# nucypher/TFHE.jl

Measured on AMD Instinct MI355X. Metric: bootstrapped gates/sec (whole node), N=1024, higher is better.
Workload: dtype int32 torus / f64 transform; 1 GPU; batch of 4096 independent gate_nand() bootstraps per GPU, tfhe_parameters_80 (n=500, N=1024, k=1, l=2, Bg=2^10, ks t=8, base 2^2); inputs=resident in HBM, launch=one process

## Files before the change

### tfhe.jl_amd/csrc/engine_dispatch.hip

```cpp
#define TFHE_EMIT_KEYSWITCH_KERNELS
#include "engine.hpp"
#include "br_launch.hpp"

#include <map>
#include <mutex>
#include <functional>

int32_t ensure_dyn_lds(tfhe_ctx *c, const void *fn, size_t bytes, const char *what)
{
    static std::mutex mu;
    static std::map<std::pair<int, const void *>, size_t> have;
    std::lock_guard<std::mutex> lk(mu);
    size_t &cur = have[std::make_pair(c->device, fn)];
    if (cur >= bytes) return TFHE_OK;
    const hipError_t e = hipFuncSetAttribute(fn, hipFuncAttributeMaxDynamicSharedMemorySize, (int)bytes);
    if (e != hipSuccess) return c->set_err(TFHE_ERR_DEVICE, "hipFuncSetAttribute(%s, %zu bytes of LDS) failed: %s", what, bytes, hipGetErrorString(e));
    cur = bytes;
    return TFHE_OK;
}

int32_t prepare_diag(tfhe_ctx *c, size_t R, hipStream_t s, DiagArgs &d)
{
    d.margin_bits = nullptr; d.clk = nullptr; d.phase = nullptr;
    c->diag_rows = 0;
    if (!c->measure_margin) return TFHE_OK;
    HIP_TRY(c, c->diag.reserve(R * 24 + 64 * 8));
    HIP_TRY(c, hipMemsetAsync(c->diag.p, 0, R * 24 + 64 * 8, s));
    d.margin_bits = (unsigned long long *)c->diag.p;
    d.clk = d.margin_bits + R;
    d.phase = d.clk + 2 * R;
    c->diag_rows = R;
    return TFHE_OK;
}

void name_kernel(tfhe_ctx *c, const char *fmt, ...)
{
    char buf[128];
    va_list ap;
    va_start(ap, fmt);
    vsnprintf(buf, sizeof buf, fmt, ap);
    va_end(ap);
    c->last_kernel = buf;
}

static int br_inst_l(const tfhe_ctx *c)
{
    return (c->P.bs_l == 2 || c->P.bs_l == 3) && !c->br_rt_l ? c->P.bs_l : 0;
}

static void name_br(tfhe_ctx *c, const char *family, int L, const char *rest = "")
{
    if (L) name_kernel(c, "blind_rotate_kernel_%s<%d%s>", family, L, rest);
    else name_kernel(c, "blind_rotate_kernel_%s<0%s>(l=%d)", family, rest, c->P.bs_l);
}

static int32_t launch_blind_rotate_part(tfhe_ctx *c, size_t first, size_t R, int32_t mu, hipStream_t s, const DiagArgs &diag, int k2_kind = -1 ,
                                        const TvPtrs *tv_all = nullptr)
{
    TvPtrs tv{nullptr, nullptr};
    if (tv_all) tv = TvPtrs{tv_all->tv, tv_all->index + first, tv_all->bodies ? tv_all->bodies + first * (size_t)tv_all->n_out : nullptr, tv_all->n_out};
    BrArgs a;
    a.diag = diag;
    if (diag.margin_bits) { a.diag.margin_bits += first; a.diag.clk += 2 * first; }
    const bool dg = c->measure_margin;
    a.bara = (const int32_t *)c->bara.p + first * (size_t)(c->P.n + 1);
    a.bk = c->d_bk;
    a.ext = (int32_t *)c->ext.p + first * ((size_t)c->P.k * c->P.N + 1);
    a.T = c->T;
    a.tan2 = reinterpret_cast<const double *>(c->d_tables + kTan2TableOffset);
    a.g = c->g;
    a.n = c->P.n;
    a.mu = mu;
    a.prio_steps = (int32_t)((int64_t)c->P.n * c->br_prio_pct / 100);
    a.R = (int32_t)R;
    const int L = c->P.bs_l;
    a.l = L;
    if (c->anyn()) {
        const int K1 = c->P.k + 1, N = c->P.N, M = N / 2;
        anyn::Args g;
        g.diag = a.diag; g.bara = a.bara; g.bk = a.bk; g.ext = a.ext; g.g = c->g; g.n = a.n; g.mu = mu; g.K1 = K1; g.L = L; g.R = (int32_t)R;
        g.log2N = ilog2i(N); g.parties = 1;
        g.wtab = c->d_anyn_tab; g.twist = c->d_anyn_tab + M;
        HIP_TRY(c, c->mk_acc.reserve((first + R) * (size_t)K1 * N * sizeof(int32_t)));
        g.acc = (int32_t *)c->mk_acc.p + first * (size_t)K1 * N;
        const bool fits = anyn::lds_bytes(N, K1) <= 160 * 1024;
        const bool spec_lds = c->anyn_spec < 0 ? fits : (c->anyn_spec == 0 && fits);
        g.spec_g = nullptr;
        if (!spec_lds) {
            HIP_TRY(c, c->spec.reserve((first + R) * (size_t)K1 * (M > 0 ? M : 1) * sizeof(cplx)));
            g.spec_g = (cplx *)c->spec.p + first * (size_t)K1 * (M > 0 ? M : 1);
        }
        const BrLaunch geo{0, 1, dg, dim3((unsigned)R), dim3((unsigned)anyn::threads_for(N)), anyn::lds_bytes(N, spec_lds ? K1 : 0)};
        const int32_t rc = tv_all ? br_launch_anyn(c, with_tv(g, tv), geo, s) : br_launch_anyn(c, g, geo, s);
        if (rc) return rc;
        name_kernel(c, spec_lds ? "blind_rotate_kernel_anyn(N=%d,k=%d,l=%d)" : "blind_rotate_kernel_anyn(N=%d,k=%d,l=%d,spec=global)", N, c->P.k, L);
        return TFHE_OK;
    }
    if (c->n512()) {
        N512Args b;
        b.diag = a.diag; b.bara = a.bara; b.bk = a.bk; b.ext = a.ext; b.g = c->g; b.n = a.n; b.mu = mu; b.R = (int32_t)R; b.l = L;
        b.prio_steps = a.prio_steps;
        b.tw1 = c->d_tables + kN512TableOffset; b.tw2q = c->d_tables + kH2TableOffset + 512; b.tw3q = b.tw2q + 64;
        if (c->n512_w2 == 1 || (c->n512_w2 < 0 && R <= 6 * (size_t)c->cu_count)) {
            const BrLaunch geo{br_inst_l(c), 1, dg, dim3((unsigned)R), dim3(128), kN512W2LdsBytes};
            const int32_t rc = tv_all ? br_launch_n512w2(c, with_tv(b, tv), geo, s) : br_launch_n512w2(c, b, geo, s);
            if (rc) return rc;
            name_br(c, "n512w2", geo.L);
            return TFHE_OK;
        }
        const bool group = !dg && (c->n512_rw == 4 || (c->n512_rw == 0 && R >= 8 * (size_t)c->cu_count));
        const int rw = group ? 4 : 1;
        const BrLaunch geo{br_inst_l(c), rw, dg, dim3((unsigned)((R + rw - 1) / rw)), dim3(64 * rw), (size_t)rw * kN512LdsBytes};
        const int32_t rc = tv_all ? br_launch_n512(c, with_tv(b, tv), geo, s) : br_launch_n512(c, b, geo, s);
        if (rc) return rc;
        name_br(c, "n512", geo.L, group ? ",rw4" : "");
        return TFHE_OK;
    }
    const bool tuned = c->P.N == kN2 ? (c->P.k == 1 && L == 3) : c->P.k == 1 ? true : (c->P.k == 2 && (L == 2 || L == 3));
    if (!tuned || c->br_general) {
        const int K1 = c->P.k + 1, H = c->P.N / kN;
        const size_t img = (size_t)kMir + c->P.N;
        BrGenArgs g;
        g.diag = a.diag; g.bara = a.bara; g.bk = a.bk; g.ext = a.ext; g.g = c->g; g.n = a.n; g.mu = mu; g.K1 = K1; g.L = L; g.R = (int32_t)R;
        HIP_TRY(c, c->mk_acc.reserve((first + R) * K1 * img * sizeof(int32_t)));
        g.acc = (int32_t *)c->mk_acc.p + first * K1 * img;
        g.tw1f = c->P.N == kN2 ? (const cplx *)(c->d_tables + kTableElems) : c->T.tw1f;
        g.tw2 = c->T.tw2;
        const BrLaunch geo{0, 1, dg, dim3((unsigned)R), dim3(64), (kXchElems + 64 + (size_t)K1 * H * kM) * sizeof(cplx)};
        const bool n2048 = c->P.N == kN2;
        const int32_t rc = tv_all ? br_launch_general(c, with_tv(g, tv), n2048, geo, s) : br_launch_general(c, g, n2048, geo, s);
        if (rc) return rc;
        name_kernel(c, "blind_rotate_kernel_general(N=%d,k=%d,l=%d)", c->P.N, c->P.k, L);
        return TFHE_OK;
    }
    if (c->P.N == kN2) {
        Br2048Args b;
        b.diag = a.diag; b.bara = a.bara; b.bk = a.bk; b.ext = a.ext; b.tw1f2 = c->d_tables + kTableElems; b.tw2 = c->T.tw2; b.g = c->g; b.n = a.n; b.mu = mu; b.prio_steps = a.prio_steps;
        b.R = (int32_t)R;
        const int rw = dg ? 1 : c->n2048_rw ? c->n2048_rw : (R <= (size_t)c->cu_count ? 1 : 2);
        const size_t ldsb = (size_t)rw * (2 * kImg2 * 4 + 2 * kXchElems * sizeof(cplx)) + 64 * sizeof(cplx) + 64;
        const BrLaunch geo{L, rw, dg, dim3((unsigned)((R + rw - 1) / rw)), dim3(128 * rw), ldsb};
        const int32_t rc = tv_all ? br_launch_n2048x(c, with_tv(b, tv), geo, s) : br_launch_n2048x(c, b, geo, s);
        if (rc) return rc;
        name_br(c, "n2048x", L, rw == 2 ? ",rw2" : ",rw1");
        return TFHE_OK;
    }
    if (c->P.k == 2) {
        const size_t cus = (size_t)c->cu_count;
        const bool w3 = k2_kind >= 0 ? k2_kind == 1 : (c->k2_w3 == 1 || (c->k2_w3 < 0 && R <= 2 * cus));
        if (w3) {
            const BrLaunch geo{L, 1, dg, dim3((unsigned)R), dim3(192), kK2W3LdsBytes};
            const int32_t rc = tv_all ? br_launch_k2w3(c, with_tv(a, tv), geo, s) : br_launch_k2w3(c, a, geo, s);
            if (rc) return rc;
            name_br(c, "k2w3", L);
            return TFHE_OK;
        }
        const bool grouped = !dg && (c->k2_rw == 7 || c->k2_rw == 0);
        size_t blocks = R;
        if (grouped) {
            const size_t rounds = (R + 7 * cus - 1) / (7 * cus);
            blocks = std::min(R, rounds * cus);
            a.grp_q = (int32_t)(R / blocks);
            a.grp_big = (int32_t)(R % blocks);
        }
        const int rw = grouped ? 7 : 1;
        const BrLaunch geo{L, rw, dg, dim3((unsigned)blocks), dim3(64 * rw), (size_t)rw * kK2LdsBytes};
        const int32_t rc = tv_all ? br_launch_k2(c, with_tv(a, tv), geo, s) : br_launch_k2(c, a, geo, s);
        if (rc) return rc;
        name_br(c, "k2", L, grouped ? ",rw7" : "");
        return TFHE_OK;
    }
    const int64_t tiny = c->br_tiny == -2 ? (int64_t)c->cu_count : c->br_tiny;
    if (tiny >= 0 && (int64_t)R <= tiny && (L == 2 || L == 3) && !c->br_rt_l) {
        H2Tables ht;
        ht.tw1h = c->d_tables + kH2TableOffset; ht.tw2q = ht.tw1h + 512; ht.tw3q = ht.tw2q + 64;
        const size_t ldsh = 2 * kImg * 4 + (size_t)4 * L * (kH2Buf + 256) * sizeof(cplx) + 2 * 2 * kN * 4;
        const BrLaunch geo{L, 1, dg, dim3((unsigned)R), dim3(256 * L), ldsh};
        const int32_t rc = tv_all ? br_launch_h2(c, with_tv(a, tv), ht, geo, s) : br_launch_h2(c, a, ht, geo, s);
        if (rc) return rc;
        name_br(c, "h2", L);
        return TFHE_OK;
    }
    if (c->br_small >= 0 && (int64_t)R <= c->br_small) {
        const size_t cus2 = 2 * (size_t)c->cu_count;
        const bool pairs = !dg && (c->w2_rw == 2 || (c->w2_rw == 0 && ((R > cus2 / 2 && R <= cus2) || R > 2 * cus2 - cus2 / 8)));
        const int rw = pairs ? 2 : 1;
        const BrLaunch geo{br_inst_l(c), rw, dg, dim3((unsigned)((R + rw - 1) / rw)), dim3(128 * rw), (size_t)rw * kW2LdsBytes};
        const int32_t rc = tv_all ? br_launch_w2(c, with_tv(a, tv), geo, s) : br_launch_w2(c, a, geo, s);
        if (rc) return rc;
        name_br(c, "w2", geo.L, pairs ? ",rw2" : "");
        return TFHE_OK;
    }
    const bool group = c->v3_rw == 4 || (c->v3_rw == 0 && R >= 6 * (size_t)c->cu_count);
    const int rw = group ? 4 : 1;
    const BrLaunch geo{br_inst_l(c), rw, dg, dim3((unsigned)((R + rw - 1) / rw)), dim3(64 * rw), (size_t)rw * kV3LdsBytes};
    const int32_t rc = tv_all ? br_launch_v3(c, with_tv(a, tv), geo, s) : br_launch_v3(c, a, geo, s);
    if (rc) return rc;
    name_br(c, "v3", geo.L, group ? ",8,tw2reg,rw4" : ",8,tw2reg");
    return TFHE_OK;
}

static const double kK2RoundCost[8] = {0.0, 6.8, 6.85, 7.2, 7.3, 9.45, 9.55, 10.3};
static const double kK2W3RoundCost[3] = {0.0, 3.1, 4.3};
struct K2Seg { size_t count; int kind; };
static std::vector<K2Seg> k2_partition(size_t R, size_t cus, bool allow_w3)
{
    const size_t q = (R + cus - 1) / cus;
    if (q <= 2 && allow_w3) return {{R, 1}};
    if (q <= 7 && !allow_w3) return {{R, 0}};
    std::vector<double> best(q + 1, 1e300);
    std::vector<int> take(q + 1, 0);
    best[0] = 0.0;
    for (size_t i = 1; i <= q; i++)
        for (int n = 1; n <= 7 && (size_t)n <= i; n++)
            if (best[i - n] + kK2RoundCost[n] < best[i]) { best[i] = best[i - n] + kK2RoundCost[n]; take[i] = n; }
    int tail = 0;
    double total = best[q];
    for (int t = 1; allow_w3 && t <= 2 && (size_t)t <= q; t++)
        if (best[q - t] + kK2W3RoundCost[t] < total) { total = best[q - t] + kK2W3RoundCost[t]; tail = t; }
    std::vector<int> rounds;
    for (size_t i = q - (size_t)tail; i > 0; i -= (size_t)take[i]) rounds.push_back(take[i]);
    std::sort(rounds.begin(), rounds.end(), std::greater<int>());
    std::vector<K2Seg> seg;
    size_t done = 0;
    for (size_t i = 0; i < rounds.size() && done < R;) {
        size_t j = i;
        while (j < rounds.size() && rounds[j] == rounds[i]) j++;
        const size_t want = (size_t)rounds[i] * (j - i) * cus;
        if ((j == rounds.size() && !tail) || done + want >= R) { seg.push_back({R - done, 0}); done = R; break; }
        seg.push_back({want, 0});
        done += want;
        i = j;
    }
    if (done < R) seg.push_back({R - done, 1});
    return seg;
}

int32_t launch_blind_rotate(tfhe_ctx *c, size_t R, int32_t mu, hipStream_t s, const TvPtrs *tv)
{
    if (tv && c->measure_margin) return c->set_err(TFHE_ERR_STATE, "bootstrap_tv: no DIAG instantiation of the TV kernels (measure_margin is on)");
    DiagArgs diag;
    int32_t rc = prepare_diag(c, R, s, diag);
    if (rc) return rc;
    alloc_checkpoint();
    std::vector<K2Seg> seg;
    const bool tuned_l = c->P.bs_l == 2 || c->P.bs_l == 3;
    if (c->anyn()) {
    } else if (c->br_split && !c->br_general && !c->measure_margin && c->P.N == kN && c->P.k == 2 && tuned_l && (c->k2_rw == 0 || c->k2_rw == 7) && c->k2_w3 != 1) {
        seg = k2_partition(R, (size_t)c->cu_count, c->k2_w3 < 0);
    } else if (c->br_split && !c->br_general && c->P.N == kN && c->P.k == 1 && c->br_small > 0) {
        const size_t resident = 8 * (size_t)c->cu_count;
        if (R > resident && R % resident > 0 && R % resident <= (size_t)c->br_small) seg = {{R - R % resident, -1}, {R % resident, -1}};
    }
    auto part = [&](size_t first, size_t count, int kind) {
        const int32_t r = launch_blind_rotate_part(c, first, count, mu, s, diag, kind, tv);
        if (!r && tv) c->last_kernel += "+tv";
        return r;
    };
    if (seg.empty()) return part(0, R, -1);
    if (seg.size() == 1) return part(0, R, seg[0].kind);
    std::string names;
    size_t first = 0;
    for (const K2Seg &sg : seg) {
        rc = part(first, sg.count, sg.kind);
        if (rc) return rc;
        if (names.empty() || names.substr(names.rfind(" + ") == std::string::npos ? 0 : names.rfind(" + ") + 3) != c->last_kernel)
            names += (names.empty() ? "" : " + ") + c->last_kernel;
        first += sg.count;
    }
    c->last_kernel = names;
    return TFHE_OK;
}

template <class A>
static A ks_args(const tfhe_ctx *c, const int32_t *e0, const int32_t *e1, const int32_t *dst, const int32_t *ext, int32_t *out)
{
    const int P = c->ks.parties, kN = c->ks.kN, n = c->P.n;
    A a{};
    a.ext = ext; a.e0 = e0; a.e1 = e1; a.dst = dst; a.out = out;
    a.n = n; a.kN = kN;
    a.in_stride = P * kN + 1; a.in_off = 0; a.in_b = P * kN; a.out_stride = P * n + 1; a.out_off = 0; a.out_b = P * n;
    return a;
}

int32_t launch_keyswitch(tfhe_ctx *c, size_t G, const int32_t *e0, const int32_t *e1, const int32_t *dst, const int32_t *ext, int32_t *out, hipStream_t s)
{
    const KsKey &K = c->ks;
    const int P = K.parties, kN = K.kN, n = c->P.n;
    if (K.mode == 4) {
        Ks4Args a = ks_args<Ks4Args>(c, e0, e1, dst, ext, out);
        a.G = (int)G; a.wtiles = K.wtiles;
        a.kslices = (P > 1 || kN % 512 != 0) ? 1 : (G <= 512 ? 16 : c->ks_slices_large);
        if (a.kslices > 1) {
            const Ks3Args i3 = ks_args<Ks3Args>(c, e0, e1, dst, ext, out);
            hipLaunchKernelGGL(ks3_init_kernel, dim3((unsigned)G), dim3(256), 0, s, i3);
        }
        a.Gpad = (int)((G + 63) / 64 * 64);
        HIP_TRY(c, c->abar.reserve((size_t)(kN / 4) * a.Gpad * 16));
        a.abar_t = (const i32x4 *)c->abar.p;
        for (int p = 0; p < P; p++) {
            a.in_off = p * kN; a.out_off = p * n; a.add_b = (p == 0);
            a.bmat = (const i32x4 *)K.p + (size_t)p * K.per_party;
            hipLaunchKernelGGL(ks4_digits_kernel, dim3((unsigned)(a.Gpad / 32), (unsigned)(kN / 128)), dim3(128), 0, s, a, (i32x4 *)c->abar.p);
            hipLaunchKernelGGL(keyswitch_kernel_v4, dim3((unsigned)((G + 255) / 256), (unsigned)K.wtiles, (unsigned)a.kslices), dim3(256), 0, s, a);
        }
    } else if (K.mode == 3) {
        Ks3Args a = ks_args<Ks3Args>(c, e0, e1, dst, ext, out);
        a.t = c->P.ks_t; a.log2_base = 2; a.stride = K.stride; a.G = (int)G;
        a.ksp = (const int32_t *)K.p;
        hipLaunchKernelGGL(ks3_init_kernel, dim3((unsigned)G), dim3(256), 0, s, a);
        const unsigned tiles = (unsigned)((G + KS3_G - 1) / KS3_G);
        for (int p = 0; p < P; p++) {
            a.in_off = p * kN; a.out_off = p * n;
            a.ksp = (const int32_t *)K.p + (size_t)p * K.per_party;
            hipLaunchKernelGGL(keyswitch_kernel_v3, dim3(tiles * KS3_SLICES, (unsigned)((K.stride + 511) / 512)), dim3(128), 0, s, a);
        }
    } else {
        KsArgs a = ks_args<KsArgs>(c, e0, e1, dst, ext, out);
        a.t = c->P.ks_t; a.log2_base = c->P.ks_log2_base;
        for (int p = 0; p < P; p++) {
            a.in_off = p * kN; a.out_off = p * n; a.add_b = (p == 0);
            a.ks = (const int32_t *)K.p + (size_t)p * K.per_party;
            hipLaunchKernelGGL(keyswitch_kernel, dim3((unsigned)G, (unsigned)((n + 1 + 256 * KS1_WPT - 1) / (256 * KS1_WPT))), dim3(256), 0, s, a);
        }
    }
    HIP_TRY(c, hipGetLastError());
    return TFHE_OK;
}
```

### tfhe.jl_amd/csrc/kernels_keyswitch.hpp

```cpp
#pragma once
#include <hip/hip_runtime.h>

#include "../../include/tfhe_mi355x.h"
#include "br_core.hpp"

using namespace tfhe;

struct KsArgs {
    const int32_t *ext;
    const int32_t *ks;
    const int32_t *e0;
    const int32_t *e1;
    const int32_t *dst;
    int32_t *out;
    int32_t n, kN, t, log2_base;
    int32_t in_stride, in_off, in_b, out_stride, out_off, out_b;
    int32_t add_b;
};

constexpr int KS1_WPT = 4;

#ifdef TFHE_EMIT_KEYSWITCH_KERNELS
__global__ __launch_bounds__(256) void keyswitch_kernel(KsArgs P)
{
    constexpr int WPT = KS1_WPT;
    const int g = blockIdx.x;
    const int tid = threadIdx.x;
    const int n1 = P.n + 1;
    const int w0 = blockIdx.y * (256 * WPT);
    const int32_t *x0 = P.ext + (size_t)P.e0[g] * P.in_stride;
    const int e1 = P.e1 ? P.e1[g] : -1;
    const int32_t *x1 = e1 >= 0 ? P.ext + (size_t)e1 * P.in_stride : nullptr;
    const int base1 = (1 << P.log2_base) - 1;
    const uint32_t prec_offset = 1u << (32 - (1 + P.log2_base * P.t));

    uint32_t accw[WPT];
#pragma unroll
    for (int u = 0; u < WPT; u++) accw[u] = 0;

    for (int i = 0; i < P.kN; i++) {
        uint32_t ai = (uint32_t)x0[P.in_off + i];
        if (x1) ai += (uint32_t)x1[P.in_off + i];
        const int32_t aibar = (int32_t)(ai + prec_offset);
        const int32_t *rows_i = P.ks + (size_t)i * P.t * base1 * n1;
        for (int j = 1; j <= P.t; j++) {
            const int d = (aibar >> (32 - j * P.log2_base)) & base1;
            if (d != 0) {
                const int32_t *row = rows_i + (size_t)((j - 1) * base1 + (d - 1)) * n1;
#pragma unroll
                for (int u = 0; u < WPT; u++) {
                    const int wd = w0 + tid + u * 256;
                    if (wd < n1) accw[u] -= (uint32_t)row[wd];
                }
            }
        }
    }
    const size_t og = P.dst ? (size_t)P.dst[g] : (size_t)g;
    int32_t *o = P.out + og * P.out_stride;
#pragma unroll
    for (int u = 0; u < WPT; u++) {
        const int wd = w0 + tid + u * 256;
        if (wd < P.n) {
            o[P.out_off + wd] = (int32_t)accw[u];
        } else if (wd == P.n) {
            uint32_t v = accw[u];
            if (P.add_b) {
                v += (uint32_t)x0[P.in_b];
                if (x1) v += (uint32_t)x1[P.in_b] + (1u << 29);
            } else {
                v += (uint32_t)o[P.out_b];
            }
            o[P.out_b] = (int32_t)v;
        }
    }
}
#endif

constexpr int KS3_G = 16;
constexpr int KS3_SLICES = 16;

struct Ks3Args {
    const int32_t *ext;
    const int32_t *ksp;
    const int32_t *e0, *e1, *dst;
    int32_t *out;
    int32_t n, kN, t, log2_base, stride, G;
    int32_t in_stride, in_off, in_b, out_stride, out_off, out_b;
};

#ifdef TFHE_EMIT_KEYSWITCH_KERNELS
__global__ void ks3_init_kernel(Ks3Args P)
{
    const int g = blockIdx.x;
    const size_t og = P.dst ? (size_t)P.dst[g] : (size_t)g;
    int32_t *o = P.out + og * P.out_stride;
    for (int w = threadIdx.x; w < P.out_b; w += blockDim.x) o[w] = 0;
    if (threadIdx.x == 0) {
        uint32_t b = (uint32_t)P.ext[(size_t)P.e0[g] * P.in_stride + P.in_b];
        const int e1 = P.e1 ? P.e1[g] : -1;
        if (e1 >= 0) b += (uint32_t)P.ext[(size_t)e1 * P.in_stride + P.in_b] + (1u << 29);
        o[P.out_b] = (int32_t)b;
    }
}
#endif

typedef uint32_t u32x4 __attribute__((ext_vector_type(4)));

#ifdef TFHE_EMIT_KEYSWITCH_KERNELS
__global__ __launch_bounds__(128, 2) void keyswitch_kernel_v3(Ks3Args P)
{
    constexpr int G = KS3_G;
    constexpr int JH = 4;
    __shared__ int32_t abar[G][128];
    const int tid = threadIdx.x;
    const int lin = blockIdx.x;
    const int xcd = lin & 7;
    const int rest = lin >> 3;
    const int slice = xcd + 8 * (rest % (KS3_SLICES / 8));
    const int tile = rest / (KS3_SLICES / 8);
    const int wchunk = blockIdx.y;
    const int g0 = tile * G;
    const int slen = P.kN / KS3_SLICES;
    const int i0 = slice * slen;
    const int lb = P.log2_base, tl = P.t;
    const int base1 = (1 << lb) - 1;
    const uint32_t prec_offset = 1u << (32 - (1 + lb * tl));
    const int w0 = wchunk * 512 + tid * 4;
    const bool active = w0 < P.stride;
    const int wl = active ? w0 : 0;

    for (int idx = tid; idx < G * slen; idx += 128) {
        const int g = idx / slen, ii = idx % slen;
        const int gg = min(g0 + g, P.G - 1);
        uint32_t ai = (uint32_t)P.ext[(size_t)P.e0[gg] * P.in_stride + P.in_off + i0 + ii];
        const int e1 = P.e1 ? P.e1[gg] : -1;
        if (e1 >= 0) ai += (uint32_t)P.ext[(size_t)e1 * P.in_stride + P.in_off + i0 + ii];
        abar[g][ii] = (int32_t)(ai + prec_offset);
    }
    __syncthreads();

    u32x4 acc[G];
#pragma unroll
    for (int g = 0; g < G; g++) acc[g] = (u32x4)(0u);

    const size_t row_words = (size_t)P.stride;
    const int stages = slen * (tl / JH);
    auto load_stage = [&](int st, u32x4 (&r)[JH][3]) {
        const int ii = st / (tl / JH), jh = st % (tl / JH);
        const int32_t *rows = P.ksp + ((size_t)(i0 + ii) * tl + jh * JH) * base1 * row_words + wl;
#pragma unroll
        for (int j = 0; j < JH; j++)
#pragma unroll
            for (int h = 0; h < 3; h++) r[j][h] = *reinterpret_cast<const u32x4 *>(rows + (size_t)(j * 3 + h) * row_words);
    };
    auto compute_stage = [&](int st, const u32x4 (&r)[JH][3]) {
        const int ii = st / (tl / JH), jh = st % (tl / JH);
#pragma unroll
        for (int g = 0; g < G; g++) {
            const int a = __builtin_amdgcn_readfirstlane(abar[g][ii]);
#pragma unroll
            for (int j = 0; j < JH; j++) {
                const int pos = 32 - (jh * JH + j + 1) * lb;
                const uint32_t m0 = (uint32_t)((a << (31 - pos)) >> 31);
                const uint32_t m1 = (uint32_t)((a << (30 - pos)) >> 31);
                const u32x4 t = (r[j][2] & m1) | (r[j][0] & ~m1);
                const u32x4 u = r[j][1] & m1;
                acc[g] -= (t & m0) | (u & ~m0);
            }
        }
    };

    u32x4 ra[JH][3], rb[JH][3];
    load_stage(0, ra);
    for (int st = 0; st < stages; st += 2) {
        if (st + 1 < stages) load_stage(st + 1, rb);
        compute_stage(st, ra);
        if (st + 2 < stages) load_stage(st + 2, ra);
        if (st + 1 < stages) compute_stage(st + 1, rb);
    }

    if (!active) return;
#pragma unroll
    for (int g = 0; g < G; g++) {
        const int gg = g0 + g;
        if (gg >= P.G) break;
        const size_t og = P.dst ? (size_t)P.dst[gg] : (size_t)gg;
        int32_t *o = P.out + og * P.out_stride;
#pragma unroll
        for (int q = 0; q < 4; q++) {
            if (w0 + q < P.n) atomicAdd(reinterpret_cast<unsigned int *>(o + P.out_off + w0 + q), acc[g][q]);
            else if (w0 + q == P.n) atomicAdd(reinterpret_cast<unsigned int *>(o + P.out_b), acc[g][q]);
        }
    }
}
#endif

typedef int32_t i32x4 __attribute__((ext_vector_type(4)));
typedef int32_t i32x16 __attribute__((ext_vector_type(16)));

struct Ks4Args {
    const int32_t *ext;
    const i32x4 *bmat;
    const int32_t *e0, *e1, *dst;
    int32_t *out;
    int32_t n, kN, G, wtiles;
    int32_t in_stride, in_off, in_b, out_stride, out_off, out_b;
    int32_t add_b;
    const i32x4 *abar_t;
    int32_t Gpad;
    int32_t kslices;
};

__host__ __device__ inline int32_t signed_byte_plane(uint32_t v, int plane)
{
    int32_t s = 0;
    for (int p = 0; p <= plane; p++) {
        const uint32_t u = v & 255u;
        s = u >= 128u ? (int32_t)u - 256 : (int32_t)u;
        v = (v - (uint32_t)s) >> 8;
    }
    return s;
}

#ifdef TFHE_EMIT_KEYPREP_KERNELS
__global__ void ks4_prepare_kernel(const int32_t *__restrict__ ks, i32x4 *__restrict__ bmat, int n, int kN, int wtiles)
{
    const size_t idx = (size_t)blockIdx.x * blockDim.x + threadIdx.x;
    const size_t total = (size_t)kN * wtiles * 4 * 64;
    if (idx >= total) return;
    const int lane = (int)(idx & 63);
    const int plane = (int)((idx >> 6) & 3);
    const int wt = (int)((idx >> 8) % wtiles);
    const int i = (int)((idx >> 8) / wtiles);
    const int c = lane & 31, h = lane >> 5;
    const int w = wt * 32 + c;
    i32x4 frag;
    for (int q = 0; q < 4; q++) {
        const int j = 4 * h + q;
        uint32_t word = 0;
        for (int hh = 1; hh <= 3; hh++) {
            int32_t sb = 0;
            if (w <= n) sb = signed_byte_plane((uint32_t)ks[(((size_t)i * 8 + j) * 3 + (hh - 1)) * (n + 1) + w], plane);
            word |= ((uint32_t)sb & 255u) << (8 * hh);
        }
        frag[q] = (int32_t)word;
    }
    bmat[idx] = frag;
}
#endif

#ifdef TFHE_EMIT_KEYSWITCH_KERNELS
__global__ __launch_bounds__(128) void ks4_digits_kernel(Ks4Args P, i32x4 *__restrict__ abar_t)
{
    __shared__ uint32_t tile[32][129];
    const int tid = threadIdx.x;
    const int g0 = blockIdx.x * 32, i0 = blockIdx.y * 128;
    for (int g = 0; g < 32; g++) {
        const int gg = min(g0 + g, P.G - 1);
        const int32_t *r0 = P.ext + (size_t)P.e0[gg] * P.in_stride + P.in_off;
        const int e1 = P.e1 ? P.e1[gg] : -1;
        uint32_t v = (uint32_t)r0[i0 + tid];
        if (e1 >= 0) v += (uint32_t)P.ext[(size_t)e1 * P.in_stride + P.in_off + i0 + tid];
        tile[g][tid] = v + (1u << 15);
    }
    __syncthreads();
    for (int k = tid; k < 32 * 32; k += 128) {
        const int q = k >> 5, g = k & 31;
        i32x4 o;
#pragma unroll
        for (int u = 0; u < 4; u++) o[u] = (int32_t)tile[g][4 * q + u];
        abar_t[(size_t)(i0 / 4 + q) * P.Gpad + g0 + g] = o;
    }
}

__global__ __launch_bounds__(256, 2) void keyswitch_kernel_v4(Ks4Args P)
{
    constexpr int MT = 2;
    __shared__ i32x4 bst[2][4][4][64];
    const int lane = threadIdx.x & 63, wave = threadIdx.x >> 6;
    const int c = lane & 31, h = lane >> 5;
    const int wt = blockIdx.y;
    const int gbase = (blockIdx.x * 4 + wave) * (32 * MT);
    const bool wave_active = gbase < P.G;

    const i32x4 *ap[MT];
#pragma unroll
    for (int mt = 0; mt < MT; mt++) ap[mt] = P.abar_t + min(gbase + mt * 32 + c, P.Gpad - 1);

    i32x16 acc[MT][4];
#pragma unroll
    for (int mt = 0; mt < MT; mt++)
#pragma unroll
        for (int pl = 0; pl < 4; pl++)
#pragma unroll
            for (int r = 0; r < 16; r++) acc[mt][pl][r] = 0;

    const size_t bstep = (size_t)P.wtiles * 4 * 64;
    const int i_begin = (int)blockIdx.z * (P.kN / P.kslices), i_end = i_begin + P.kN / P.kslices;
    const i32x4 *bp = P.bmat + (size_t)i_begin * bstep + ((size_t)wt * 4 + wave) * 64 + lane;
    const int stages = (i_end - i_begin) / 4;
    i32x4 pre[4];
#pragma unroll
    for (int ii = 0; ii < 4; ii++) bst[0][ii][wave][lane] = bp[(size_t)ii * bstep];

    i32x4 a_cur[MT], a_nxt[MT];
    auto load_a = [&](int i4, i32x4 (&a)[MT]) {
#pragma unroll
        for (int mt = 0; mt < MT; mt++) a[mt] = ap[mt][(size_t)(i4 >> 2) * P.Gpad];
    };
    load_a(i_begin, a_cur);

    for (int st = 0; st < stages; st++) {
        const bool more = st + 1 < stages;
        if (more) {
#pragma unroll
            for (int ii = 0; ii < 4; ii++) pre[ii] = bp[(size_t)(4 * (st + 1) + ii) * bstep];
            load_a(i_begin + 4 * (st + 1), a_nxt);
        }
        __syncthreads();
        if (wave_active) {
#pragma unroll
            for (int ii = 0; ii < 4; ii++) {
                i32x4 afrag[MT];
#pragma unroll
                for (int mt = 0; mt < MT; mt++)
#pragma unroll
                    for (int q = 0; q < 4; q++) {
                        const uint32_t d8 = ((uint32_t)a_cur[mt][ii] >> (27 - 2 * (4 * h + q))) & 24u;
                        afrag[mt][q] = (int32_t)(1u << d8);
                    }
#pragma unroll
                for (int pl = 0; pl < 4; pl++) {
                    const i32x4 bfrag = bst[st & 1][ii][pl][lane];
#pragma unroll
                    for (int mt = 0; mt < MT; mt++)
                        acc[mt][pl] = __builtin_amdgcn_mfma_i32_32x32x32_i8(afrag[mt], bfrag, acc[mt][pl], 0, 0, 0);
                }
            }
        }
        if (more) {
#pragma unroll
            for (int ii = 0; ii < 4; ii++) bst[(st + 1) & 1][ii][wave][lane] = pre[ii];
#pragma unroll
            for (int mt = 0; mt < MT; mt++) a_cur[mt] = a_nxt[mt];
        }
    }
    if (!wave_active) return;

    const int w = wt * 32 + c;
    if (w > P.n) return;
#pragma unroll
    for (int mt = 0; mt < MT; mt++)
#pragma unroll
        for (int r = 0; r < 16; r++) {
            const int gg = gbase + mt * 32 + (r & 3) + 8 * (r >> 2) + 4 * h;
            if (gg >= P.G) continue;
            uint32_t sum = (uint32_t)acc[mt][0][r] + ((uint32_t)acc[mt][1][r] << 8) + ((uint32_t)acc[mt][2][r] << 16) +
                           ((uint32_t)acc[mt][3][r] << 24);
            const size_t og = P.dst ? (size_t)P.dst[gg] : (size_t)gg;
            int32_t *o = P.out + og * P.out_stride;
            if (P.kslices > 1) {
                atomicAdd(reinterpret_cast<unsigned int *>(o + (w < P.n ? P.out_off + w : P.out_b)), 0u - sum);
            } else if (w < P.n) {
                o[P.out_off + w] = (int32_t)(0u - sum);
            } else {
                if (P.add_b) {
                    uint32_t b = (uint32_t)P.ext[(size_t)P.e0[gg] * P.in_stride + P.in_b];
                    const int e1 = P.e1 ? P.e1[gg] : -1;
                    if (e1 >= 0) b += (uint32_t)P.ext[(size_t)e1 * P.in_stride + P.in_b] + (1u << 29);
                    o[P.out_b] = (int32_t)(b - sum);
                } else {
                    o[P.out_b] = (int32_t)((uint32_t)o[P.out_b] - sum);
                }
            }
        }
}
#endif
```

Measured before the change: 365,800 gates/s.

## Remap keyswitch blocks so each XCD shares key tiles, fold row init into digits kernel

```diff
diff --git a/tfhe.jl_amd/csrc/engine_dispatch.hip b/tfhe.jl_amd/csrc/engine_dispatch.hip
--- a/tfhe.jl_amd/csrc/engine_dispatch.hip
+++ b/tfhe.jl_amd/csrc/engine_dispatch.hip
@@ -290,11 +290,13 @@
     if (K.mode == 4) {
         Ks4Args a = ks_args<Ks4Args>(c, e0, e1, dst, ext, out);
         a.G = (int)G; a.wtiles = K.wtiles;
-        a.kslices = (P > 1 || kN % 512 != 0) ? 1 : (G <= 512 ? 16 : c->ks_slices_large);
-        if (a.kslices > 1) {
-            const Ks3Args i3 = ks_args<Ks3Args>(c, e0, e1, dst, ext, out);
-            hipLaunchKernelGGL(ks3_init_kernel, dim3((unsigned)G), dim3(256), 0, s, i3);
-        }
+        const bool sliced = P == 1 && kN % 512 == 0;
+        a.kslices = !sliced ? 1 : (G <= 512 ? 16 : c->ks_slices_large);
+        a.init_rows = a.kslices > 1;
+        a.xcd_order = sliced && G > 512;
+        const unsigned groups = (unsigned)((G + 255) / 256);
+        const dim3 grid4 = a.xcd_order ? dim3(ks4_block_count(groups, (unsigned)K.wtiles, (unsigned)a.kslices))
+                                       : dim3(groups, (unsigned)K.wtiles, (unsigned)a.kslices);
         a.Gpad = (int)((G + 63) / 64 * 64);
         HIP_TRY(c, c->abar.reserve((size_t)(kN / 4) * a.Gpad * 16));
         a.abar_t = (const i32x4 *)c->abar.p;
@@ -302,7 +304,7 @@
             a.in_off = p * kN; a.out_off = p * n; a.add_b = (p == 0);
             a.bmat = (const i32x4 *)K.p + (size_t)p * K.per_party;
             hipLaunchKernelGGL(ks4_digits_kernel, dim3((unsigned)(a.Gpad / 32), (unsigned)(kN / 128)), dim3(128), 0, s, a, (i32x4 *)c->abar.p);
-            hipLaunchKernelGGL(keyswitch_kernel_v4, dim3((unsigned)((G + 255) / 256), (unsigned)K.wtiles, (unsigned)a.kslices), dim3(256), 0, s, a);
+            hipLaunchKernelGGL(keyswitch_kernel_v4, grid4, dim3(256), 0, s, a);
         }
     } else if (K.mode == 3) {
         Ks3Args a = ks_args<Ks3Args>(c, e0, e1, dst, ext, out);
diff --git a/tfhe.jl_amd/csrc/kernels_keyswitch.hpp b/tfhe.jl_amd/csrc/kernels_keyswitch.hpp
--- a/tfhe.jl_amd/csrc/kernels_keyswitch.hpp
+++ b/tfhe.jl_amd/csrc/kernels_keyswitch.hpp
@@ -3,6 +3,7 @@
 
 #include "../../include/tfhe_mi355x.h"
 #include "br_core.hpp"
+#include "ks4_block_order.hpp"
 
 using namespace tfhe;
 
@@ -209,6 +210,8 @@
     const i32x4 *abar_t;
     int32_t Gpad;
     int32_t kslices;
+    int32_t init_rows;
+    int32_t xcd_order;
 };
 
 __host__ __device__ inline int32_t signed_byte_plane(uint32_t v, int plane)
@@ -271,6 +274,21 @@
         for (int u = 0; u < 4; u++) o[u] = (int32_t)tile[g][4 * q + u];
         abar_t[(size_t)(i0 / 4 + q) * P.Gpad + g0 + g] = o;
     }
+    if (P.init_rows) {
+        const int lane = tid & 63, ny = (int)gridDim.y;
+        for (int g = (int)blockIdx.y + ny * (tid >> 6); g < 32 && g0 + g < P.G; g += ny * 2) {
+            const int gg = g0 + g;
+            const size_t og = P.dst ? (size_t)P.dst[gg] : (size_t)gg;
+            int32_t *o = P.out + og * P.out_stride;
+            for (int w = lane; w < P.out_b; w += 64) o[w] = 0;
+            if (lane == 0) {
+                uint32_t b = (uint32_t)P.ext[(size_t)P.e0[gg] * P.in_stride + P.in_b];
+                const int e1 = P.e1 ? P.e1[gg] : -1;
+                if (e1 >= 0) b += (uint32_t)P.ext[(size_t)e1 * P.in_stride + P.in_b] + (1u << 29);
+                o[P.out_b] = (int32_t)b;
+            }
+        }
+    }
 }
 
 __global__ __launch_bounds__(256, 2) void keyswitch_kernel_v4(Ks4Args P)
@@ -279,8 +297,14 @@
     __shared__ i32x4 bst[2][4][4][64];
     const int lane = threadIdx.x & 63, wave = threadIdx.x >> 6;
     const int c = lane & 31, h = lane >> 5;
-    const int wt = blockIdx.y;
-    const int gbase = (blockIdx.x * 4 + wave) * (32 * MT);
+    int sgroup = blockIdx.x, wt = blockIdx.y, slice = blockIdx.z;
+    if (P.xcd_order) {
+        constexpr int GS = 4 * 32 * MT;
+        const Ks4Block k = ks4_block_of(blockIdx.x, (unsigned)((P.G + GS - 1) / GS), (unsigned)P.wtiles, (unsigned)P.kslices);
+        if (k.group < 0) return;
+        sgroup = k.group; wt = k.wtile; slice = k.slice;
+    }
+    const int gbase = (sgroup * 4 + wave) * (32 * MT);
     const bool wave_active = gbase < P.G;
 
     const i32x4 *ap[MT];
@@ -296,7 +320,7 @@
             for (int r = 0; r < 16; r++) acc[mt][pl][r] = 0;
 
     const size_t bstep = (size_t)P.wtiles * 4 * 64;
-    const int i_begin = (int)blockIdx.z * (P.kN / P.kslices), i_end = i_begin + P.kN / P.kslices;
+    const int i_begin = slice * (P.kN / P.kslices), i_end = i_begin + P.kN / P.kslices;
     const i32x4 *bp = P.bmat + (size_t)i_begin * bstep + ((size_t)wt * 4 + wave) * 64 + lane;
     const int stages = (i_end - i_begin) / 4;
     i32x4 pre[4];
diff --git a/tfhe.jl_amd/csrc/ks4_block_order.hpp b/tfhe.jl_amd/csrc/ks4_block_order.hpp
--- /dev/null
+++ b/tfhe.jl_amd/csrc/ks4_block_order.hpp
@@ -0,0 +1,28 @@
+#pragma once
+
+#if defined(__HIPCC__)
+#define KS4_HD __host__ __device__ inline
+#else
+#define KS4_HD inline
+#endif
+
+constexpr unsigned KS4_XCDS = 8;
+
+struct Ks4Block { int group, wtile, slice; };
+
+KS4_HD unsigned ks4_block_count(unsigned groups, unsigned wtiles, unsigned kslices)
+{
+    const unsigned pairs = wtiles * kslices;
+    return (pairs + KS4_XCDS - 1) / KS4_XCDS * KS4_XCDS * groups;
+}
+
+KS4_HD Ks4Block ks4_block_of(unsigned b, unsigned groups, unsigned wtiles, unsigned kslices)
+{
+    const unsigned x = b % KS4_XCDS, q = b / KS4_XCDS;
+    const unsigned pair = q / groups * KS4_XCDS + x;
+    Ks4Block r;
+    r.group = pair < wtiles * kslices ? (int)(q % groups) : -1;
+    r.wtile = (int)(pair / kslices);
+    r.slice = (int)(pair % kslices);
+    return r;
+}
```

Result: no change. 367,500 gates/s, median of 6 (+0.5%).
